# hby1320/pytorch_object_detection

Measured on AMD Instinct MI355X. Metric: images/sec HISFCOS-R50 640x640 inference, higher is better.
Workload: dtype f32

## Files before the change

pytorch_object_detection_amd/csrc/fd_stem.hip:

```cpp
#include "fd_conv_common.h"

#define ST_TH 8
#define ST_TW 32
#define ST_PR (2 * ST_TH + 5)
#define ST_PC (2 * ST_TW + 5)
#define ST_PITCH 208
#define ST_KR 22
#define ST_CO 64
#define ST_TPW 4

struct StemArgs {
    const float4* x; const float* xp;
    const float* w; const float* scale; const float* shift; float* y;
    int y_cs, y_co, N, H, W, Ho, Wo, act, tiles_h, tiles_w;
};

template <bool POOL, bool NCHW>
__global__ __launch_bounds__(256, 2) void stem7x7_kernel(StemArgs a) {
    extern __shared__ __attribute__((aligned(16))) char smem[];
    float* Ws = reinterpret_cast<float*>(smem);
    float* Ps = Ws + 7 * ST_KR * ST_CO;
    float* St = Ps + ST_PR * ST_PITCH;
    float* Cb = Ps;
    float* Cy = St + 4 * 1024;
    const int tid = threadIdx.x, lane = tid & 63, wave = tid >> 6;
    const int l31 = lane & 31, lh = lane >> 5;
    for (int i = tid; i < 7 * ST_KR * ST_CO / 4; i += 256)
        reinterpret_cast<float4*>(Ws)[i] = reinterpret_cast<const float4*>(a.w)[i];
    if (tid < ST_PR) Ps[tid * ST_PITCH + ST_PITCH - 1] = 0.f;

    constexpr int NPX = (ST_PR * ST_PC + 255) / 256;
    float4 pv[NPX];
    const int ntile = a.N * a.tiles_h * a.tiles_w;
    auto tile_pos = [&](int t, int& n, int& ho0, int& wo0) {
        if constexpr (POOL) {
            const int th = t % a.tiles_h; t /= a.tiles_h;
            const int tw = t % a.tiles_w;
            n = t / a.tiles_w; ho0 = th * ST_TH; wo0 = tw * ST_TW;
        } else {
            const int tw = t % a.tiles_w; t /= a.tiles_w;
            const int th = t % a.tiles_h;
            n = t / a.tiles_h; ho0 = th * ST_TH; wo0 = tw * ST_TW;
        }
    };
    auto load_patch = [&](int t) {
        int n, ho0, wo0;
        tile_pos(t, n, ho0, wo0);
        const size_t HW = (size_t)a.H * a.W;
        const float4* xin = a.x + (size_t)n * HW;
        const float* xpl = a.xp + (size_t)n * 3 * HW;
#pragma unroll
        for (int u = 0; u < NPX; ++u) {
            const int i = tid + 256 * u;
            const int pr = i / ST_PC, pc = i - pr * ST_PC;
            const int hi = 2 * ho0 - 3 + pr, wi = 2 * wo0 - 3 + pc;
            pv[u] = make_float4(0.f, 0.f, 0.f, 0.f);
            if (i < ST_PR * ST_PC && (unsigned)hi < (unsigned)a.H && (unsigned)wi < (unsigned)a.W) {
                if constexpr (NCHW) {
                    const float* q = xpl + (size_t)hi * a.W + wi;
                    pv[u].x = q[0]; pv[u].y = q[HW]; pv[u].z = q[2 * HW];
                } else {
                    pv[u] = xin[(size_t)hi * a.W + wi];
                }
            }
        }
    };
    auto store_patch = [&]() {
#pragma unroll
        for (int u = 0; u < NPX; ++u) {
            const int i = tid + 256 * u;
            if (i < ST_PR * ST_PC) {
                const int pr = i / ST_PC, pc = i - pr * ST_PC;
                float* d = Ps + pr * ST_PITCH + pc * 3;
                d[0] = pv[u].x; d[1] = pv[u].y; d[2] = pv[u].z;
            }
        }
    };

    const int t0 = blockIdx.x * ST_TPW, t1 = min(ntile, t0 + ST_TPW);
    load_patch(t0);
    store_patch();
    __syncthreads();
    const float* A0 = Ps + (2 * (2 * wave)) * ST_PITCH + (2 * l31) * 3 + lh;
    const float* A1 = A0 + 2 * ST_PITCH;
    const float* B0 = Ws + lh * ST_CO + l31;
    float* stage = St + wave * 1024;
    for (int t = t0; t < t1; ++t) {
        int n, ho0, wo0;
        tile_pos(t, n, ho0, wo0);
        if (t + 1 < t1) load_patch(t + 1);
        f32x16 acc[2][2];
#pragma unroll
        for (int i = 0; i < 2; ++i)
#pragma unroll
            for (int j = 0; j < 2; ++j)
#pragma unroll
                for (int e = 0; e < 16; ++e) acc[i][j][e] = 0.f;
        constexpr int NSTEP = 7 * (ST_KR / 2);
        float a0 = A0[0], a1 = A1[0], b0 = B0[0], b1 = B0[32];
#pragma unroll
        for (int s_ = 0; s_ < NSTEP; ++s_) {
            float a0n = 0.f, a1n = 0.f, b0n = 0.f, b1n = 0.f;
            if (s_ + 1 < NSTEP) {
                const int r = (s_ + 1) / (ST_KR / 2), jj = (s_ + 1) % (ST_KR / 2);
                a0n = A0[r * ST_PITCH + 2 * jj]; a1n = A1[r * ST_PITCH + 2 * jj];
                b0n = B0[(r * ST_KR + 2 * jj) * ST_CO]; b1n = B0[(r * ST_KR + 2 * jj) * ST_CO + 32];
            }
            __builtin_amdgcn_sched_barrier(0);
            acc[0][0] = __builtin_amdgcn_mfma_f32_32x32x2f32(a0, b0, acc[0][0], 0, 0, 0);
            acc[0][1] = __builtin_amdgcn_mfma_f32_32x32x2f32(a0, b1, acc[0][1], 0, 0, 0);
            acc[1][0] = __builtin_amdgcn_mfma_f32_32x32x2f32(a1, b0, acc[1][0], 0, 0, 0);
            acc[1][1] = __builtin_amdgcn_mfma_f32_32x32x2f32(a1, b1, acc[1][1], 0, 0, 0);
            __builtin_amdgcn_sched_barrier(0);
            a0 = a0n; a1 = a1n; b0 = b0n; b1 = b1n;
        }
        __syncthreads();
        if constexpr (POOL) {
            const bool first = (t == t0), last = (t + 1 == t1);
            const int Hp = (a.Ho - 1) / 2 + 1, Wp = (a.Wo - 1) / 2 + 1;
#pragma unroll
            for (int j = 0; j < 2; ++j) {
                const int nn0 = j * 32;
                const float sc = a.scale ? a.scale[nn0 + l31] : 1.0f;
                const float sf = a.shift ? a.shift[nn0 + l31] : 0.0f;
#pragma unroll
                for (int i = 0; i < 2; ++i) {
                    const int row = 2 * wave + i;
                    const bool rok = ho0 + row < a.Ho;
#pragma unroll
                    for (int e = 0; e < 16; ++e) {
                        const int col = (e & 3) + 8 * (e >> 2) + 4 * lh;
                        const float v = acc[i][j][e] * sc + sf;
                        Cb[(row * 32 + col) * 32 + l31] = (rok && wo0 + col < a.Wo && v > 0.f) ? v : 0.f;
                    }
                }
                __syncthreads();
                for (int it = tid; it < 5 * 17 * 8; it += 256) {
                    const int c4 = it & 7, pc = (it >> 3) % 17, pr = (it >> 3) / 17;
                    const int cr = 2 * pr, cc = 2 * pc;
                    if (pr == 4 && !last) continue;
                    const int ph = (ho0 + cr) >> 1, pw = (wo0 + cc) >> 1;
                    if (ph >= Hp || pw >= Wp) continue;
                    float4 m = make_float4(0.f, 0.f, 0.f, 0.f);
#pragma unroll
                    for (int dr = -1; dr <= 1; ++dr) {
                        const int r = cr + dr;
                        if (r > 7) continue;
                        if (r < 0 && first) continue;
#pragma unroll
                        for (int dc = -1; dc <= 1; ++dc) {
                            const int c = cc + dc;
                            if (c < 0 || c > 31) continue;
                            const float4 v = r < 0 ? *reinterpret_cast<const float4*>(Cy + c * 64 + nn0 + c4 * 4)
                                                   : *reinterpret_cast<const float4*>(Cb + (r * 32 + c) * 32 + c4 * 4);
                            m.x = fmaxf(m.x, v.x); m.y = fmaxf(m.y, v.y); m.z = fmaxf(m.z, v.z); m.w = fmaxf(m.w, v.w);
                        }
                    }
                    const bool whole = (pr < 4) && (cr > 0 || !first || ho0 == 0) && (pc < 16) && (cc > 0 || wo0 == 0);
                    float* yp = a.y + ((size_t)(n * Hp + ph) * Wp + pw) * a.y_cs + a.y_co + nn0 + c4 * 4;
                    if (whole) {
                        *reinterpret_cast<float4*>(yp) = m;
                    } else {
                        unsigned* up = reinterpret_cast<unsigned*>(yp);
                        atomicMax(up + 0, __float_as_uint(m.x)); atomicMax(up + 1, __float_as_uint(m.y));
                        atomicMax(up + 2, __float_as_uint(m.z)); atomicMax(up + 3, __float_as_uint(m.w));
                    }
                }
                const float4 cyv = *reinterpret_cast<const float4*>(Cb + (7 * 32 + (tid >> 3)) * 32 + (tid & 7) * 4);
                __syncthreads();
                if (!last) *reinterpret_cast<float4*>(Cy + (tid >> 3) * 64 + nn0 + (tid & 7) * 4) = cyv;
            }
            __syncthreads();
            if (tid < ST_PR) Ps[tid * ST_PITCH + ST_PITCH - 1] = 0.f;
            if (t + 1 < t1) store_patch();
        } else {
        if (t + 1 < t1) store_patch();
#pragma unroll
        for (int j = 0; j < 2; ++j) {
            const int nn0 = j * 32;
            const float sc = a.scale ? a.scale[nn0 + l31] : 1.0f;
            const float sf = a.shift ? a.shift[nn0 + l31] : 0.0f;
#pragma unroll
            for (int i = 0; i < 2; ++i) {
                const int ho = ho0 + 2 * wave + i;
#pragma unroll
                for (int e = 0; e < 16; ++e)
                    stage[((e & 3) + 8 * (e >> 2) + 4 * lh) * 32 + l31] = fd_act1(acc[i][j][e] * sc + sf, a.act, 0.f);
                wave_lds_sync();
#pragma unroll
                for (int p = 0; p < 4; ++p) {
                    const int row = (lane >> 3) + 8 * p, c4 = (lane & 7) * 4;
                    const int wo = wo0 + row;
                    if (ho < a.Ho && wo < a.Wo) {
                        const float4 v = *reinterpret_cast<const float4*>(stage + row * 32 + c4);
                        *reinterpret_cast<float4*>(a.y + ((size_t)(n * a.Ho + ho) * a.Wo + wo) * a.y_cs + a.y_co + nn0 + c4) = v;
                    }
                }
                wave_lds_sync();
            }
        }
        }
        __syncthreads();
    }
}

__global__ __launch_bounds__(256) void stem_pool_zero_kernel(float* __restrict__ y, int y_cs, int y_co, int N, int Hp, int Wp) {
    constexpr int RS = ST_TH * ST_TPW / 2, CS = ST_TW / 2;
    const int nrows = (Hp - 1) / RS, ncols = (Wp - 1) / CS;
    const int per_img = nrows * Wp + Hp * ncols;
    const long total = (long)N * per_img * 16;
    for (long i = (long)blockIdx.x * 256 + threadIdx.x; i < total; i += (long)gridDim.x * 256) {
        const int c4 = (int)(i & 15);
        const long q = i >> 4;
        const int n = (int)(q / per_img);
        int r = (int)(q - (long)n * per_img), ph, pw;
        if (r < nrows * Wp) { ph = RS * (1 + r / Wp); pw = r % Wp; }
        else { r -= nrows * Wp; ph = r / ncols; pw = CS * (1 + r % ncols); }
        *reinterpret_cast<float4*>(y + (((long)n * Hp + ph) * Wp + pw) * y_cs + y_co + c4 * 4) = make_float4(0.f, 0.f, 0.f, 0.f);
    }
}

static int stem_launch(bool pool, bool nchw, const float* x4, const float* w, const float* scale, const float* shift, float* y, int32_t y_cs, int32_t y_co, int32_t N,
                       int32_t H, int32_t W, int32_t act, hipStream_t stream) {
    FD_REQUIRE(x4 && w && y && N >= 1 && H >= 2 && W >= 2, FD_E_INVAL, "fd_stem7x7: bad arguments");
    FD_REQUIRE(((((nchw ? (uintptr_t)0 : (uintptr_t)x4)) | (uintptr_t)w | (uintptr_t)y) & 15) == 0 && ((uintptr_t)x4 & 3) == 0 && y_cs % 4 == 0 && y_co % 4 == 0 &&
                   y_cs >= y_co + ST_CO, FD_E_INVAL, "fd_stem7x7: pointers must be 16-byte aligned (the NCHW planes: 4-byte) and the 64-channel output view 4-aligned");
    FD_REQUIRE(act == FD_ACT_NONE || act == FD_ACT_RELU || act == FD_ACT_SILU, FD_E_INVAL, "fd_stem7x7: activation none / ReLU / SiLU");
    StemArgs a;
    a.x = reinterpret_cast<const float4*>(x4); a.xp = x4; a.w = w; a.scale = scale; a.shift = shift; a.y = y;
    a.y_cs = y_cs; a.y_co = y_co; a.N = N; a.H = H; a.W = W; a.act = act;
    a.Ho = (H + 6 - 7) / 2 + 1; a.Wo = (W + 6 - 7) / 2 + 1;
    a.tiles_h = (a.Ho + ST_TH - 1) / ST_TH; a.tiles_w = (a.Wo + ST_TW - 1) / ST_TW;
    const long out_rows = pool ? (long)N * ((a.Ho - 1) / 2 + 1) * ((a.Wo - 1) / 2 + 1) : (long)N * a.Ho * a.Wo;
    FD_REQUIRE(out_rows * y_cs < (1L << 31), FD_E_UNSUPPORTED, "fd_stem7x7: tensor exceeds 2^31 elements");
    if (pool) {
        a.tiles_h = (a.tiles_h + ST_TPW - 1) / ST_TPW * ST_TPW;
        const long blocks = (long)N * a.tiles_w * (a.tiles_h / ST_TPW);
        FD_REQUIRE(blocks < (1L << 31), FD_E_UNSUPPORTED, "fd_stem7x7: too many tiles");
        constexpr int lds = (7 * ST_KR * ST_CO + ST_PR * ST_PITCH + 4 * 1024 + 32 * 64) * 4;
        static std::atomic<unsigned> attr_mask{0}, attr_mask_p{0};
        if (nchw) fd_set_max_lds_once(attr_mask_p, reinterpret_cast<const void*>(stem7x7_kernel<true, true>), lds);
        else fd_set_max_lds_once(attr_mask, reinterpret_cast<const void*>(stem7x7_kernel<true, false>), lds);
        {
            const int Hp = (a.Ho - 1) / 2 + 1, Wp = (a.Wo - 1) / 2 + 1;
            const long items = (long)N * (((Hp - 1) / (ST_TH * ST_TPW / 2)) * Wp + Hp * ((Wp - 1) / (ST_TW / 2))) * 16;
            long g = (items + 255) / 256;
            if (g > 8192) g = 8192;
            if (g > 0) hipLaunchKernelGGL(stem_pool_zero_kernel, dim3((unsigned)g), dim3(256), 0, stream, y, y_cs, y_co, N, Hp, Wp);
            FD_CHECK_LAUNCH("fd_stem7x7_pool_nhwc4 (zero)");
        }
        if (nchw) hipLaunchKernelGGL((stem7x7_kernel<true, true>), dim3((unsigned)blocks), dim3(256), lds, stream, a);
        else hipLaunchKernelGGL((stem7x7_kernel<true, false>), dim3((unsigned)blocks), dim3(256), lds, stream, a);
        FD_CHECK_LAUNCH("fd_stem7x7 (+ max-pool)");
        return FD_OK;
    }
    const long blocks = ((long)N * a.tiles_h * a.tiles_w + ST_TPW - 1) / ST_TPW;
    FD_REQUIRE(blocks < (1L << 31), FD_E_UNSUPPORTED, "fd_stem7x7: too many tiles");
    constexpr int lds = (ST_PR * ST_PITCH + 7 * ST_KR * ST_CO + 4 * 1024) * 4;
    static std::atomic<unsigned> attr_mask{0}, attr_mask_p{0};
    if (nchw) {
        fd_set_max_lds_once(attr_mask_p, reinterpret_cast<const void*>(stem7x7_kernel<false, true>), lds);
        hipLaunchKernelGGL((stem7x7_kernel<false, true>), dim3((unsigned)blocks), dim3(256), lds, stream, a);
    } else {
        fd_set_max_lds_once(attr_mask, reinterpret_cast<const void*>(stem7x7_kernel<false, false>), lds);
        hipLaunchKernelGGL((stem7x7_kernel<false, false>), dim3((unsigned)blocks), dim3(256), lds, stream, a);
    }
    FD_CHECK_LAUNCH("fd_stem7x7");
    return FD_OK;
}

extern "C" int32_t fd_stem7x7_nhwc4(const float* x4, const float* w, const float* scale, const float* shift, float* y, int32_t y_cs,
                                    int32_t y_co, int32_t N, int32_t H, int32_t W, int32_t act, fd_stream_t stream_) {
    return stem_launch(false, false, x4, w, scale, shift, y, y_cs, y_co, N, H, W, act, (hipStream_t)stream_);
}

extern "C" int32_t fd_stem7x7_pool_nhwc4(const float* x4, const float* w, const float* scale, const float* shift, float* y_pooled, int32_t y_cs,
                                         int32_t y_co, int32_t N, int32_t H, int32_t W, fd_stream_t stream_) {
    return stem_launch(true, false, x4, w, scale, shift, y_pooled, y_cs, y_co, N, H, W, FD_ACT_RELU, (hipStream_t)stream_);
}

extern "C" int32_t fd_stem7x7_nchw3(const float* x, const float* w, const float* scale, const float* shift, float* y, int32_t y_cs, int32_t y_co,
                                    int32_t N, int32_t H, int32_t W, int32_t act, int32_t pool, fd_stream_t stream_) {
    FD_REQUIRE((long)N * 3 * H * W < (1L << 31), FD_E_UNSUPPORTED, "fd_stem7x7_nchw3: input exceeds 2^31 elements");
    return stem_launch(pool != 0, true, x, w, scale, shift, y, y_cs, y_co, N, H, W, pool ? FD_ACT_RELU : act, (hipStream_t)stream_);
}
```

Before: 1438.

## Fuse stem max-pool in registers using cross-wave row exchange and lane shuffles

Rewrites the fused 3x3/2 max-pool epilogue of the 7x7 stem. It drops the LDS staging of the whole conv tile and the per-channel-half loop with its extra barriers. Each wave now does BN+ReLU in registers, swaps one boundary row with the neighbouring wave through a small LDS buffer, and does the horizontal pooling with cross-half lane shuffles, writing scalars straight to global memory. It also hoists the scale/shift loads out of the tile loop, shrinks the LDS footprint, and adds optional compile-time timestamp probes. The scalar stores are less coalesced than the old float4 writes, and the edge and atomic handling is intricate.

```diff
diff --git a/pytorch_object_detection_amd/csrc/fd_stem.hip b/pytorch_object_detection_amd/csrc/fd_stem.hip
--- a/pytorch_object_detection_amd/csrc/fd_stem.hip
+++ b/pytorch_object_detection_amd/csrc/fd_stem.hip
@@ -13,7 +13,16 @@
     const float4* x; const float* xp;
     const float* w; const float* scale; const float* shift; float* y;
     int y_cs, y_co, N, H, W, Ho, Wo, act, tiles_h, tiles_w;
+#ifdef FD_STEM_TIMING
+    long long* ts;
+#endif
 };
+
+#ifdef FD_STEM_TIMING
+#define ST_TS(k) do { if (a.ts && threadIdx.x == 0) a.ts[((size_t)blockIdx.x * ST_TPW + (t - t0)) * 8 + (k)] = wall_clock64(); } while (0)
+#else
+#define ST_TS(k) do { } while (0)
+#endif
 
 template <bool POOL, bool NCHW>
 __global__ __launch_bounds__(256, 2) void stem7x7_kernel(StemArgs a) {
@@ -21,8 +30,7 @@
     float* Ws = reinterpret_cast<float*>(smem);
     float* Ps = Ws + 7 * ST_KR * ST_CO;
     float* St = Ps + ST_PR * ST_PITCH;
-    float* Cb = Ps;
-    float* Cy = St + 4 * 1024;
+    float* Rx = St;
     const int tid = threadIdx.x, lane = tid & 63, wave = tid >> 6;
     const int l31 = lane & 31, lh = lane >> 5;
     for (int i = tid; i < 7 * ST_KR * ST_CO / 4; i += 256)
@@ -85,9 +93,20 @@
     const float* A1 = A0 + 2 * ST_PITCH;
     const float* B0 = Ws + lh * ST_CO + l31;
     float* stage = St + wave * 1024;
+    const int Hp = (a.Ho - 1) / 2 + 1, Wp = (a.Wo - 1) / 2 + 1;
+    float psc[2] = {1.0f, 1.0f}, psf[2] = {0.0f, 0.0f};
+    const unsigned loff = (unsigned)(2 * lh * a.y_cs + l31);
+    if constexpr (POOL) {
+#pragma unroll
+        for (int j = 0; j < 2; ++j) {
+            if (a.scale) psc[j] = a.scale[j * 32 + l31];
+            if (a.shift) psf[j] = a.shift[j * 32 + l31];
+        }
+    }
     for (int t = t0; t < t1; ++t) {
         int n, ho0, wo0;
         tile_pos(t, n, ho0, wo0);
+        ST_TS(0);
         if (t + 1 < t1) load_patch(t + 1);
         f32x16 acc[2][2];
 #pragma unroll
@@ -114,63 +133,93 @@
             __builtin_amdgcn_sched_barrier(0);
             a0 = a0n; a1 = a1n; b0 = b0n; b1 = b1n;
         }
+        ST_TS(1);
         __syncthreads();
         if constexpr (POOL) {
+            ST_TS(2);
             const bool first = (t == t0), last = (t + 1 == t1);
-            const int Hp = (a.Ho - 1) / 2 + 1, Wp = (a.Wo - 1) / 2 + 1;
-#pragma unroll
-            for (int j = 0; j < 2; ++j) {
-                const int nn0 = j * 32;
-                const float sc = a.scale ? a.scale[nn0 + l31] : 1.0f;
-                const float sf = a.shift ? a.shift[nn0 + l31] : 0.0f;
-#pragma unroll
-                for (int i = 0; i < 2; ++i) {
-                    const int row = 2 * wave + i;
-                    const bool rok = ho0 + row < a.Ho;
-#pragma unroll
-                    for (int e = 0; e < 16; ++e) {
-                        const int col = (e & 3) + 8 * (e >> 2) + 4 * lh;
-                        const float v = acc[i][j][e] * sc + sf;
-                        Cb[(row * 32 + col) * 32 + l31] = (rok && wo0 + col < a.Wo && v > 0.f) ? v : 0.f;
-                    }
-                }
-                __syncthreads();
-                for (int it = tid; it < 5 * 17 * 8; it += 256) {
-                    const int c4 = it & 7, pc = (it >> 3) % 17, pr = (it >> 3) / 17;
-                    const int cr = 2 * pr, cc = 2 * pc;
-                    if (pr == 4 && !last) continue;
-                    const int ph = (ho0 + cr) >> 1, pw = (wo0 + cc) >> 1;
-                    if (ph >= Hp || pw >= Wp) continue;
-                    float4 m = make_float4(0.f, 0.f, 0.f, 0.f);
-#pragma unroll
-                    for (int dr = -1; dr <= 1; ++dr) {
-                        const int r = cr + dr;
-                        if (r > 7) continue;
-                        if (r < 0 && first) continue;
-#pragma unroll
-                        for (int dc = -1; dc <= 1; ++dc) {
-                            const int c = cc + dc;
-                            if (c < 0 || c > 31) continue;
-                            const float4 v = r < 0 ? *reinterpret_cast<const float4*>(Cy + c * 64 + nn0 + c4 * 4)
-                                                   : *reinterpret_cast<const float4*>(Cb + (r * 32 + c) * 32 + c4 * 4);
-                            m.x = fmaxf(m.x, v.x); m.y = fmaxf(m.y, v.y); m.z = fmaxf(m.z, v.z); m.w = fmaxf(m.w, v.w);
+            const int ti = t - t0;
+            if (ho0 + ST_TH <= a.Ho && wo0 + ST_TW <= a.Wo) {
+#pragma unroll
+                for (int j = 0; j < 2; ++j)
+#pragma unroll
+                    for (int i = 0; i < 2; ++i)
+#pragma unroll
+                        for (int e = 0; e < 16; ++e) {
+                            const float v = acc[i][j][e] * psc[j] + psf[j];
+                            acc[i][j][e] = v > 0.f ? v : 0.f;
+                        }
+            } else {
+                const int clim = a.Wo - wo0 - 4 * lh;
+#pragma unroll
+                for (int j = 0; j < 2; ++j)
+#pragma unroll
+                    for (int i = 0; i < 2; ++i) {
+                        const bool rok = ho0 + 2 * wave + i < a.Ho;
+#pragma unroll
+                        for (int e = 0; e < 16; ++e) {
+                            const float v = acc[i][j][e] * psc[j] + psf[j];
+                            const bool keep = rok & ((e & 3) + 8 * (e >> 2) < clim) & (v > 0.f);
+                            acc[i][j][e] = keep ? v : 0.f;
                         }
                     }
-                    const bool whole = (pr < 4) && (cr > 0 || !first || ho0 == 0) && (pc < 16) && (cc > 0 || wo0 == 0);
-                    float* yp = a.y + ((size_t)(n * Hp + ph) * Wp + pw) * a.y_cs + a.y_co + nn0 + c4 * 4;
-                    if (whole) {
-                        *reinterpret_cast<float4*>(yp) = m;
-                    } else {
-                        unsigned* up = reinterpret_cast<unsigned*>(yp);
-                        atomicMax(up + 0, __float_as_uint(m.x)); atomicMax(up + 1, __float_as_uint(m.y));
-                        atomicMax(up + 2, __float_as_uint(m.z)); atomicMax(up + 3, __float_as_uint(m.w));
+            }
+            {
+                float4* Rw = reinterpret_cast<float4*>(wave < 3 ? (wave == 0 ? Rx : Ps + (wave - 1) * 2048) : Rx + (1 + (ti & 1)) * 2048) + lane;
+#pragma unroll
+                for (int j = 0; j < 2; ++j)
+#pragma unroll
+                    for (int g = 0; g < 4; ++g)
+                        Rw[(j * 4 + g) * 64] = make_float4(acc[1][j][4 * g], acc[1][j][4 * g + 1], acc[1][j][4 * g + 2], acc[1][j][4 * g + 3]);
+            }
+            __syncthreads();
+            ST_TS(3);
+            auto hpool = [&](const f32x16 (&vals)[2], int ph, bool row_atomic) {
+                if (ph >= Hp) return;
+                float* rowp = a.y + ((size_t)(n * Hp + ph) * Wp + (wo0 >> 1)) * a.y_cs + a.y_co;
+                const int pcs = Wp - (wo0 >> 1);
+                auto emit = [&](float val, int pc, int j, bool atomic) {
+                    if (pcs < 17 && pc + 2 * lh >= pcs) return;
+                    float* yp = rowp + (pc * a.y_cs + j * 32) + loff;
+                    if (atomic) atomicMax(reinterpret_cast<unsigned*>(yp), __float_as_uint(val));
+                    else *yp = val;
+                };
+#pragma unroll
+                for (int j = 0; j < 2; ++j) {
+                    float nbr[4];
+#pragma unroll
+                    for (int g = 0; g < 4; ++g) nbr[g] = __shfl_xor(vals[j][4 * g + 3], 32);
+#pragma unroll
+                    for (int g = 0; g < 4; ++g) {
+                        const float left = lh ? nbr[g] : (g ? nbr[(g + 3) & 3] : 0.f);
+                        const float pa = fmaxf(fmaxf(left, vals[j][4 * g]), vals[j][4 * g + 1]);
+                        const float pb = fmaxf(fmaxf(vals[j][4 * g + 1], vals[j][4 * g + 2]), vals[j][4 * g + 3]);
+                        emit(pa, 4 * g, j, row_atomic || (g == 0 && lh == 0 && wo0 != 0));
+                        emit(pb, 4 * g + 1, j, row_atomic);
                     }
+                    if (lh) emit(vals[j][15], 16 - 2, j, true);
                 }
-                const float4 cyv = *reinterpret_cast<const float4*>(Cb + (7 * 32 + (tid >> 3)) * 32 + (tid & 7) * 4);
-                __syncthreads();
-                if (!last) *reinterpret_cast<float4*>(Cy + (tid >> 3) * 64 + nn0 + (tid & 7) * 4) = cyv;
-            }
+            };
+            if (last && wave == 3) hpool(acc[1], (ho0 >> 1) + 4, true);
+            if (wave > 0 || !first) {
+                const float4* Rr = reinterpret_cast<const float4*>(wave > 0 ? (wave == 1 ? Rx : Ps + (wave - 2) * 2048) : Rx + (1 + ((ti - 1) & 1)) * 2048) + lane;
+#pragma unroll
+                for (int j = 0; j < 2; ++j)
+#pragma unroll
+                    for (int g = 0; g < 4; ++g) {
+                        const float4 u = Rr[(j * 4 + g) * 64];
+                        acc[1][j][4 * g] = fmaxf(acc[1][j][4 * g], u.x); acc[1][j][4 * g + 1] = fmaxf(acc[1][j][4 * g + 1], u.y);
+                        acc[1][j][4 * g + 2] = fmaxf(acc[1][j][4 * g + 2], u.z); acc[1][j][4 * g + 3] = fmaxf(acc[1][j][4 * g + 3], u.w);
+                    }
+            }
+#pragma unroll
+            for (int j = 0; j < 2; ++j)
+#pragma unroll
+                for (int e = 0; e < 16; ++e) acc[1][j][e] = fmaxf(acc[1][j][e], acc[0][j][e]);
+            hpool(acc[1], (ho0 >> 1) + wave, wave == 0 && first && ho0 != 0);
+            ST_TS(4);
             __syncthreads();
+            ST_TS(5);
             if (tid < ST_PR) Ps[tid * ST_PITCH + ST_PITCH - 1] = 0.f;
             if (t + 1 < t1) store_patch();
         } else {
@@ -201,6 +250,7 @@
         }
         }
         __syncthreads();
+        ST_TS(6);
     }
 }
 
@@ -220,14 +270,26 @@
     }
 }
 
+#ifdef FD_STEM_TIMING
+#define ST_TS_CAP (1L << 20)
+static long long* st_ts_dev = nullptr;
+static long st_ts_n = 0;
+extern "C" int64_t fd_stem_timing_stamps(long long* out, int64_t cap) {
+    if (!st_ts_dev || st_ts_n > cap) return -1;
+    if (hipDeviceSynchronize() != hipSuccess) return -1;
+    if (hipMemcpy(out, st_ts_dev, st_ts_n * sizeof(long long), hipMemcpyDeviceToHost) != hipSuccess) return -1;
+    return st_ts_n;
+}
+#endif
+
 static int stem_launch(bool pool, bool nchw, const float* x4, const float* w, const float* scale, const float* shift, float* y, int32_t y_cs, int32_t y_co, int32_t N,
                        int32_t H, int32_t W, int32_t act, hipStream_t stream) {
     FD_REQUIRE(x4 && w && y && N >= 1 && H >= 2 && W >= 2, FD_E_INVAL, "fd_stem7x7: bad arguments");
     FD_REQUIRE(((((nchw ? (uintptr_t)0 : (uintptr_t)x4)) | (uintptr_t)w | (uintptr_t)y) & 15) == 0 && ((uintptr_t)x4 & 3) == 0 && y_cs % 4 == 0 && y_co % 4 == 0 &&
                    y_cs >= y_co + ST_CO, FD_E_INVAL, "fd_stem7x7: pointers must be 16-byte aligned (the NCHW planes: 4-byte) and the 64-channel output view 4-aligned");
     FD_REQUIRE(act == FD_ACT_NONE || act == FD_ACT_RELU || act == FD_ACT_SILU, FD_E_INVAL, "fd_stem7x7: activation none / ReLU / SiLU");
-    StemArgs a;
-    a.x = reinterpret_cast<const float4*>(x4); a.xp = x4; a.w = w; a.scale = scale; a.shift = shift; a.y = y;
+    StemArgs a = {};
+    a.x =reinterpret_cast<const float4*>(x4); a.xp = x4; a.w = w; a.scale = scale; a.shift = shift; a.y = y;
     a.y_cs = y_cs; a.y_co = y_co; a.N = N; a.H = H; a.W = W; a.act = act;
     a.Ho = (H + 6 - 7) / 2 + 1; a.Wo = (W + 6 - 7) / 2 + 1;
     a.tiles_h = (a.Ho + ST_TH - 1) / ST_TH; a.tiles_w = (a.Wo + ST_TW - 1) / ST_TW;
@@ -237,7 +299,13 @@
         a.tiles_h = (a.tiles_h + ST_TPW - 1) / ST_TPW * ST_TPW;
         const long blocks = (long)N * a.tiles_w * (a.tiles_h / ST_TPW);
         FD_REQUIRE(blocks < (1L << 31), FD_E_UNSUPPORTED, "fd_stem7x7: too many tiles");
-        constexpr int lds = (7 * ST_KR * ST_CO + ST_PR * ST_PITCH + 4 * 1024 + 32 * 64) * 4;
+        constexpr int lds = (7 * ST_KR * ST_CO + ST_PR * ST_PITCH + 3 * 2048) * 4;
+#ifdef FD_STEM_TIMING
+        if (blocks * ST_TPW * 8 <= ST_TS_CAP) {
+            if (!st_ts_dev) (void)hipMalloc((void**)&st_ts_dev, ST_TS_CAP * sizeof(long long));
+            if (st_ts_dev) { a.ts = st_ts_dev; st_ts_n = blocks * ST_TPW * 8; (void)hipMemsetAsync(st_ts_dev, 0, st_ts_n * sizeof(long long), stream); }
+        }
+#endif
         static std::atomic<unsigned> attr_mask{0}, attr_mask_p{0};
         if (nchw) fd_set_max_lds_once(attr_mask_p, reinterpret_cast<const void*>(stem7x7_kernel<true, true>), lds);
         else fd_set_max_lds_once(attr_mask, reinterpret_cast<const void*>(stem7x7_kernel<true, false>), lds);
```

Measured after the change: 1449, median of 6. Within noise of the previous version (+0.8%).
